# tlepoint/fhe.rs

Measured on NVIDIA H100. Metric: bfv_ct_mul_relin_per_sec_n32768_14x62bit, higher is better.
Workload: dtype u64

## Files before the change

### fhe_rs_b200/csrc/kernels.cu

```cuda
#include <algorithm>
#include <cstdint>
#include <cstdlib>
#include <cstring>

#include "engine.hpp"
#include "ntt_tma.cuh"

namespace fhe_b200 {

typedef unsigned __int128 u128;

namespace {

struct EwArgs {
  u64* a;
  const u64* b;
  size_t n_words;
  u32 logn, limbs_per_poly;
  const LimbDev* limbs;
  unsigned short ids[kMaxPos];
};

template <int OP>
__global__ void ew_kernel(EwArgs A) {
// ... 174 lines not shown
  size_t idx = (size_t)blockIdx.x * blockDim.x + threadIdx.x;
  size_t total = ((size_t)A.cts * nc * K) << A.logn;
  if (idx >= total) return;
  const u32 c = idx & (N - 1);
  size_t row = idx >> A.logn;
  const u32 pos = row % K;
  row /= K;
  const u32 k = row % nc, ct = (u32)(row / nc);
  const LimbDev& M = A.limbs[A.ids[pos]];
  const bool ext = pos >= A.L;
  const u32 rows = ext ? A.E : A.L, r = ext ? pos - A.L : pos;
  const u64* pa = (ext ? A.xa : A.a) + ((((size_t)ct * A.na) * rows + r) << A.logn) + c;
  const u64* pb = (ext ? A.xb : A.b) + ((((size_t)ct * A.nb) * rows + r) << A.logn) + c;
  const size_t ps = (size_t)rows << A.logn;
  Acc192 acc;
  acc.clear();
  const u32 lo = k + 1 > A.nb ? k + 1 - A.nb : 0, hi = k < A.na - 1 ? k : A.na - 1;
  for (u32 i = lo; i <= hi; i++) acc.mac(pa[i * ps], pb[(k - i) * ps]);
  A.out[idx] = acc.reduce(M);
}

struct ScaleArgs {
  ScalerDev S;
  const LimbDev* limbs;
  const u64* in;
  u64 *out0, *out1;
  u32 polys, out_rows_per_poly, start, n_out, split3, logn;
};

struct U256 {
  u64 w0, w1, w2, w3;
};
__device__ __forceinline__ U256 u256_from_acc(const u32 (&a)[7]) {
  U256 r;
  r.w0 = ((u64)a[1] << 32) | a[0];
  r.w1 = ((u64)a[3] << 32) | a[2];
  r.w2 = ((u64)a[5] << 32) | a[4];
  r.w3 = a[6];
  return r;
}
__device__ __forceinline__ U256 u256_add(U256 a, U256 b) {
  U256 r;
  asm("add.cc.u64 %0, %4, %8;\n\t"
      "addc.cc.u64 %1, %5, %9;\n\t"
      "addc.cc.u64 %2, %6, %10;\n\t"
      "addc.u64 %3, %7, %11;"
      : "=l"(r.w0), "=l"(r.w1), "=l"(r.w2), "=l"(r.w3)
      : "l"(a.w0), "l"(a.w1), "l"(a.w2), "l"(a.w3), "l"(b.w0), "l"(b.w1), "l"(b.w2), "l"(b.w3));
  return r;
}
__device__ __forceinline__ U256 u256_sub(U256 a, U256 b) {
  U256 r;
  asm("sub.cc.u64 %0, %4, %8;\n\t"
      "subc.cc.u64 %1, %5, %9;\n\t"
      "subc.cc.u64 %2, %6, %10;\n\t"
      "subc.u64 %3, %7, %11;"
      : "=l"(r.w0), "=l"(r.w1), "=l"(r.w2), "=l"(r.w3)
      : "l"(a.w0), "l"(a.w1), "l"(a.w2), "l"(a.w3), "l"(b.w0), "l"(b.w1), "l"(b.w2), "l"(b.w3));
  return r;
}
__device__ __forceinline__ U256 u256_mul_128(u128 v, u64 tlo, u64 thi) {
  u32 a[7] = {0, 0, 0, 0, 0, 0, 0}, b[7] = {0, 0, 0, 0, 0, 0, 0};
  mac_theta(a, (u64)v, tlo, thi);
  mac_theta(b, (u64)(v >> 64), tlo, thi);
  U256 lo = u256_from_acc(a), hi = u256_from_acc(b);
  U256 hs = {0, hi.w0, hi.w1, hi.w2};
  return u256_add(lo, hs);
}

constexpr int kScaleTC = 128;

__device__ __forceinline__ void stage_omega_split(u32* s_om, const ScalerDev& S, u32 start, u32 n_out, u32 n_out4) {
  const u32 nf = S.n_from;
  for (u32 idx = threadIdx.x; idx < nf * n_out4; idx += blockDim.x) {
    const u32 ii = idx / n_out4, jj = idx - ii * n_out4;
    const Split31 w = split31(jj < n_out ? S.omega[(size_t)(start + jj) * nf + ii] : 0);
    u32* row = s_om + (size_t)ii * 3 * n_out4 + jj;
    row[0] = w.lo;
    row[n_out4] = w.hi;
    row[2 * n_out4] = w.sum;
  }
}

template <int G, int UNR = 2>
__device__ __forceinline__ void scale_mac_group(AccKara (&acc)[4], const u64* r_col, const u32* om, u32 nf,
                                                u32 n_out4) {
#pragma unroll UNR
  for (u32 i = 0; i < nf; i++) {
    const Split31 r = split31(r_col[i * kScaleTC]);
    const u32* row = om + (size_t)i * 3 * n_out4;
    const uint4 w0 = *reinterpret_cast<const uint4*>(row);
    const uint4 w1 = *reinterpret_cast<const uint4*>(row + n_out4);
    const uint4 ws = *reinterpret_cast<const uint4*>(row + 2 * n_out4);
    acc[0].mac(r.lo, r.hi, r.sum, w0.x, w1.x, ws.x);
    if (G > 1) acc[1].mac(r.lo, r.hi, r.sum, w0.y, w1.y, ws.y);
    if (G > 2) acc[2].mac(r.lo, r.hi, r.sum, w0.z, w1.z, ws.z);
    if (G > 3) acc[3].mac(r.lo, r.hi, r.sum, w0.w, w1.w, ws.w);
  }
}

__global__ void __launch_bounds__(kScaleTC) scale_kernel(ScaleArgs A) {
  extern __shared__ __align__(16) u64 smem[];
  const ScalerDev& S = A.S;
  const u32 nf = S.n_from, n_out = A.n_out;
  const u32 n_out4 = (n_out + 3) & ~3u;
  constexpr u32 TC = kScaleTC;
  u64* s_r = smem;
  u32* s_omega = reinterpret_cast<u32*>(s_r + (size_t)nf * TC);
  u64* s_gamma = reinterpret_cast<u64*>(s_omega + (size_t)nf * 3 * n_out4);
  u64* s_tgl = s_gamma + n_out4;
  u64* s_tgh = s_tgl + nf;
  u64* s_tol = s_tgh + nf;
  u64* s_toh = s_tol + nf;
  u32* s_ord = reinterpret_cast<u32*>(s_toh + nf);

  const u32 N = 1u << A.logn;
  const u32 per_poly = N / TC;
  const u32 poly = blockIdx.x / per_poly;
  const u32 c0 = (blockIdx.x % per_poly) * TC;
  const u64* src = A.in + (((size_t)poly * nf) << A.logn) + c0;
  const u32 cc = threadIdx.x;

  {
    const u32 dst0 = (u32)__cvta_generic_to_shared(s_r + cc);
    for (u32 i = 0; i < nf; i++)
      asm volatile("cp.async.ca.shared.global [%0], [%1], 8;" ::"r"(dst0 + i * TC * 8u),
                   "l"(src + ((size_t)i << A.logn) + cc)
                   : "memory");
    asm volatile("cp.async.commit_group;" ::: "memory");
  }
  stage_omega_split(s_omega, S, A.start, n_out, n_out4);
  for (u32 i = cc; i < n_out4; i += TC) s_gamma[i] = i < n_out ? S.gamma[A.start + i] : 0;
  for (u32 i = cc; i < nf; i += TC) {
    s_tgl[i] = S.tgar_lo[i];
    s_tgh[i] = S.tgar_hi[i];
    s_tol[i] = S.to_lo[i];
    s_toh[i] = S.to_hi[i];
    s_ord[i] = i < S.n_terms ? S.to_order[i] : 0;
  }
  asm volatile("cp.async.wait_all;" ::: "memory");
  __syncthreads();

  u128 v;
  {
    AccTheta at;
    at.clear();
#pragma unroll 2
    for (u32 i = 0; i < nf; i++) at.mac(s_r[i * TC + cc], s_tgl[i], s_tgh[i]);
    u32 acc[7];
    at.words(acc);
    U256 sg = u256_from_acc(acc);
    const u32 bs = S.shift - 1 - 64;
    u64 lo = (sg.w1 >> bs) | (sg.w2 << (64 - bs));
    u64 hi = (sg.w2 >> bs) | (sg.w3 << (64 - bs));
    u128 x = ((u128)hi << 64) | lo;
    v = (x >> 1) + (x & 1);
  }
  bool w_sign = false;
  u128 w = 0;
  if (!S.is_one) {
    U256 s_pos = {0, 0, 0, 0}, s_neg = {0, 0, 0, 0};
#pragma unroll 1
    for (u32 sg = 0; sg < 2; sg++) {
      AccTheta at;
      at.clear();
      const u32 k0 = sg ? S.n_pos : 0, k1 = sg ? S.n_terms : S.n_pos;
#pragma unroll 2
      for (u32 k = k0; k < k1; k++) {
        const u32 i = s_ord[k];
        at.mac(s_r[i * TC + cc], s_tol[i], s_toh[i]);
      }
      u32 wds[7];
      at.words(wds);
      if (sg == 0) s_pos = u256_from_acc(wds);
      else s_neg = u256_from_acc(wds);
    }
    U256 so = u256_sub(s_pos, s_neg);
    U256 vt = u256_mul_128(v, S.tg_lo, S.tg_hi);
    so = S.tg_sign ? u256_add(so, vt) : u256_sub(so, vt);
    w_sign = (so.w3 != 0) || (so.w2 >> 63);
    if (w_sign) {
      u64 n1 = ~so.w1, n2 = ~so.w2, n3 = ~so.w3;
      u128 y = ((u128)((n2 >> 62) | (n3 << 2)) << 64) | ((n1 >> 62) | (n2 << 2));
      w = (y + 1) >> 1;
    } else {
      u128 y = ((u128)((so.w2 >> 62) | (so.w3 << 2)) << 64) | ((so.w1 >> 62) | (so.w2 << 2));
      w = (y >> 1) + (y & 1);
    }
  }

  for (u32 j0 = 0; j0 < n_out; j0 += 4) {
    AccKara acc[4];
#pragma unroll
    for (int k = 0; k < 4; k++) acc[k].clear();
    const u32* om = s_omega + j0;
    switch (min(4u, n_out - j0)) {
      case 4: scale_mac_group<4>(acc, s_r + cc, om, nf, n_out4); break;
      case 3: scale_mac_group<3>(acc, s_r + cc, om, nf, n_out4); break;
      case 2: scale_mac_group<2>(acc, s_r + cc, om, nf, n_out4); break;
      default: scale_mac_group<1>(acc, s_r + cc, om, nf, n_out4); break;
    }
#pragma unroll
    for (int k = 0; k < 4; k++) {
      const u32 jj = j0 + k;
      if (jj >= n_out) break;
      const LimbDev& M = A.limbs[S.to_ids[A.start + jj]];
      u64 vr = reduce94_limb((u64)v, (u64)(v >> 64), M);
      acc[k].mac(split31(vr ? M.p - vr : 0), split31(s_gamma[jj]));
      if (!S.is_one) {
        u64 wr = reduce94_limb((u64)w, (u64)(w >> 64), M);
        acc[k].add64(w_sign ? (wr ? M.p - wr : 0) : wr);
      }
      u64 y = acc[k].reduce(M);
      u64* dst;
      if (A.split3) {
        u32 ct = poly / 3, part = poly % 3;
        dst = part < 2 ? A.out0 + ((((size_t)ct * 2 + part) * n_out + jj) << A.logn)
                       : A.out1 + (((size_t)ct * n_out + jj) << A.logn);
      } else {
        dst = A.out0 + (((size_t)poly * A.out_rows_per_poly + jj) << A.logn);
      }
      dst[c0 + cc] = y;
    }
  }
}


struct ScaleTmaArgs {
  ScalerDev S;
  const LimbDev* limbs;
  u64 *out0, *out1;
  u32 polys, out_rows_per_poly, start, n_out, split3, logn;
  u32 tiles_total;
};

template <bool IS_ONE, int UNR>
__global__ void __launch_bounds__(kScaleTC) scale_tma_kernel(const __grid_constant__ CUtensorMap tm_in, const ScaleTmaArgs A) {
  using namespace tma;
  extern __shared__ __align__(128) u64 smem[];
  const ScalerDev& S = A.S;
  const u32 nf = S.n_from, n_out = A.n_out;
  const u32 n_out4 = (n_out + 3) & ~3u;
  constexpr u32 TC = kScaleTC;
  u64* s_r = smem;
  u32* s_omega = reinterpret_cast<u32*>(s_r + (size_t)nf * TC);
  u64* s_gamma = reinterpret_cast<u64*>(s_omega + (size_t)nf * 3 * n_out4);
  u64* s_p2 = s_gamma + n_out4;
  u64* s_c = s_p2 + n_out4;
  u64* s_tgl = s_c + n_out4;
  u64* s_tgh = s_tgl + nf;
  u64* s_tol = s_tgh + nf;
  u64* s_toh = s_tol + nf;
  u32* s_ord = reinterpret_cast<u32*>(s_toh + nf);
  u64* s_bar = reinterpret_cast<u64*>(s_ord + ((nf + 1) & ~1u));
  const u32 bar = smem_u32(s_bar);
  const u32 cc = threadIdx.x;

  stage_omega_split(s_omega, S, A.start, n_out, n_out4);
  for (u32 i = cc; i < n_out4; i += TC) {
    const bool live = i < n_out;
    const LimbDev& M = A.limbs[S.to_ids[A.start + (live ? i : 0)]];
    s_gamma[i] = live ? S.gamma[A.start + i] : 0;
    s_p2[i] = M.p2;
    s_c[i] = M.sol_c;
  }
  for (u32 i = cc; i < nf; i += TC) {
    s_tgl[i] = S.tgar_lo[i];
    s_tgh[i] = S.tgar_hi[i];
    const u32 src = (!IS_ONE && i < S.n_terms) ? S.to_order[i] : 0;
    s_tol[i] = IS_ONE ? 0 : S.to_lo[src];
    s_toh[i] = IS_ONE ? 0 : S.to_hi[src];
    s_ord[i] = src * TC * 8;
  }
  if (cc == 0) {
    mbar_init(bar, 1);
    asm volatile("fence.mbarrier_init.release.cluster;" ::: "memory");
  }
  __syncthreads();

  const u32 N = 1u << A.logn;
  const u32 per_poly = N / TC;
  const u32 dst_r = smem_u32(s_r);
  const u32 tile_bytes = nf * TC * 8;
  u32 tile = blockIdx.x;
  if (cc == 0 && tile < A.tiles_total) {
    mbar_expect_tx(bar, tile_bytes);
    load_2d(dst_r, &tm_in, (tile % per_poly) * TC, (tile / per_poly) * nf, bar);
  }
  const u32 my_r = dst_r + cc * 8;
  for (u32 it = 0; tile < A.tiles_total; tile += gridDim.x, it++) {
    const u32 poly = tile / per_poly;
    const u32 c0 = (tile - poly * per_poly) * TC;
    mbar_wait(bar, it & 1);

    u128 v;
    {
      AccTheta at;
      at.clear();
#pragma unroll 2
      for (u32 i = 0; i < nf; i++) at.mac(lds64(my_r + i * TC * 8), s_tgl[i], s_tgh[i]);
      u32 acc[7];
      at.words(acc);
      U256 sg = u256_from_acc(acc);
      const u32 bs = S.shift - 1 - 64;
      u64 lo = (sg.w1 >> bs) | (sg.w2 << (64 - bs));
      u64 hi = (sg.w2 >> bs) | (sg.w3 << (64 - bs));
      u128 x = ((u128)hi << 64) | lo;
      v = (x >> 1) + (x & 1);
    }
    bool w_sign = false;
    u128 w = 0;
    if (!IS_ONE) {
      U256 s_pos = {0, 0, 0, 0}, s_neg = {0, 0, 0, 0};
#pragma unroll 1
      for (u32 sg = 0; sg < 2; sg++) {
        AccTheta at;
        at.clear();
        const u32 k0 = sg ? S.n_pos : 0, k1 = sg ? S.n_terms : S.n_pos;
#pragma unroll 2
        for (u32 k = k0; k < k1; k++) at.mac(lds64(my_r + s_ord[k]), s_tol[k], s_toh[k]);
        u32 wds[7];
        at.words(wds);
        if (sg == 0) s_pos = u256_from_acc(wds);
        else s_neg = u256_from_acc(wds);
      }
      U256 so = u256_sub(s_pos, s_neg);
      U256 vt = u256_mul_128(v, S.tg_lo, S.tg_hi);
      so = S.tg_sign ? u256_add(so, vt) : u256_sub(so, vt);
      w_sign = (so.w3 != 0) || (so.w2 >> 63);
      if (w_sign) {
        u64 n1 = ~so.w1, n2 = ~so.w2, n3 = ~so.w3;
        u128 y = ((u128)((n2 >> 62) | (n3 << 2)) << 64) | ((n1 >> 62) | (n2 << 2));
        w = (y + 1) >> 1;
      } else {
        u128 y = ((u128)((so.w2 >> 62) | (so.w3 << 2)) << 64) | ((so.w1 >> 62) | (so.w2 << 2));
        w = (y >> 1) + (y & 1);
      }
    }
    const u64 mask62 = (1ull << 62) - 1;
    const u64 vl = (u64)v & mask62, wl = (u64)w & mask62;
    const u32 vh = (u32)(v >> 62), wh = (u32)(w >> 62);

    u64* dst;
    size_t dstride = (size_t)1 << A.logn;
    if (A.split3) {
      const u32 ct = poly / 3, part = poly - ct * 3;
      dst = part < 2 ? A.out0 + ((((size_t)ct * 2 + part) * n_out) << A.logn) : A.out1 + (((size_t)ct * n_out) << A.logn);
    } else {
      dst = A.out0 + (((size_t)poly * A.out_rows_per_poly) << A.logn);
    }
    dst += c0 + cc;

    for (u32 j0 = 0; j0 < n_out; j0 += 4) {
      AccKara acc[4];
#pragma unroll
      for (int k = 0; k < 4; k++) acc[k].clear();
      const u32* om = s_omega + j0;
      const u32 g = min(4u, n_out - j0);
      switch (g) {
        case 4: scale_mac_group<4, UNR>(acc, s_r + cc, om, nf, n_out4); break;
        case 3: scale_mac_group<3, UNR>(acc, s_r + cc, om, nf, n_out4); break;
        case 2: scale_mac_group<2, UNR>(acc, s_r + cc, om, nf, n_out4); break;
        default: scale_mac_group<1, UNR>(acc, s_r + cc, om, nf, n_out4); break;
      }
      if (j0 + 4 >= n_out) {
        __syncthreads();
        const u32 nxt = tile + gridDim.x;
        if (cc == 0 && nxt < A.tiles_total) {
          mbar_expect_tx(bar, tile_bytes);
          load_2d(dst_r, &tm_in, (nxt % per_poly) * TC, (nxt / per_poly) * nf, bar);
        }
      }
#pragma unroll
      for (int k = 0; k < 4; k++) {
        const u32 jj = j0 + k;
        if (jj >= n_out) break;
        const u64 p2 = s_p2[jj];
        const u32 c = (u32)s_c[jj];
        acc[k].mac(split31(csub(p2 - ((u64)vh * c + vl), p2 >> 1)), split31(s_gamma[jj]));
        if (!IS_ONE) {
          const u64 wr = (u64)wh * c + wl;
          acc[k].add64(w_sign ? p2 - wr : wr);
        }
        u64 lo, mid;
        u32 hi32;
        acc[k].merged(lo, mid, hi32);
        dst[(size_t)jj * dstride] = csub(fold192_solinas(lo, mid, hi32, c), p2 >> 1);
      }
    }
  }
}

__global__ void scale_small_kernel(ScaleArgs A) {
  const ScalerDev& S = A.S;
  const u32 nf = S.n_from, n_out = A.n_out;
  const u32 N = 1u << A.logn;
  const u32 idx = blockIdx.x * blockDim.x + threadIdx.x;
  if (idx >= A.polys * N) return;
  const u32 poly = idx >> A.logn, c = idx & (N - 1);
  const u64* src = A.in + (((size_t)poly * nf) << A.logn) + c;
  u32 av[7] = {0, 0, 0, 0, 0, 0, 0}, ap[7] = {0, 0, 0, 0, 0, 0, 0}, an[7] = {0, 0, 0, 0, 0, 0, 0};
  for (u32 i = 0; i < nf; i++) {
    const u64 r = src[(size_t)i << A.logn];
    mac_theta(av, r, S.tgar_lo[i], S.tgar_hi[i]);
    if (!S.is_one) {
      if (S.to_sign[i]) mac_theta(an, r, S.to_lo[i], S.to_hi[i]);
      else mac_theta(ap, r, S.to_lo[i], S.to_hi[i]);
    }
  }
  U256 sg = u256_from_acc(av);
  const u32 bs = S.shift - 1 - 64;
  u64 lo = (sg.w1 >> bs) | (sg.w2 << (64 - bs));
  u64 hi = (sg.w2 >> bs) | (sg.w3 << (64 - bs));
  u128 x = ((u128)hi << 64) | lo;
  u128 v = (x >> 1) + (x & 1);
  bool w_sign = false;
  u128 w = 0;
  if (!S.is_one) {
    U256 so = u256_sub(u256_from_acc(ap), u256_from_acc(an));
    U256 vt = u256_mul_128(v, S.tg_lo, S.tg_hi);
    so = S.tg_sign ? u256_add(so, vt) : u256_sub(so, vt);
    w_sign = (so.w3 != 0) || (so.w2 >> 63);
    if (w_sign) {
      u64 n1 = ~so.w1, n2 = ~so.w2, n3 = ~so.w3;
      u128 y = ((u128)((n2 >> 62) | (n3 << 2)) << 64) | ((n1 >> 62) | (n2 << 2));
      w = (y + 1) >> 1;
    } else {
      u128 y = ((u128)((so.w2 >> 62) | (so.w3 << 2)) << 64) | ((so.w1 >> 62) | (so.w2 << 2));
      w = (y >> 1) + (y & 1);
    }
  }
  for (u32 j = 0; j < n_out; j++) {
    const LimbDev& M = A.limbs[S.to_ids[A.start + j]];
    Acc192 acc;
    acc.clear();
    for (u32 i = 0; i < nf; i++) acc.mac(src[(size_t)i << A.logn], S.omega[(size_t)(A.start + j) * nf + i]);
    u64 vr = reduce128_limb((u64)v, (u64)(v >> 64), M);
    acc.mac(vr ? M.p - vr : 0, S.gamma[A.start + j]);
    if (!S.is_one) {
      u64 wr = reduce128_limb((u64)w, (u64)(w >> 64), M);
      acc.add64(w_sign ? (wr ? M.p - wr : 0) : wr);
    }
    u64 y = acc.reduce(M);
    u64* dst;
    if (A.split3) {
      u32 ct = poly / 3, part = poly % 3;
      dst = part < 2 ? A.out0 + ((((size_t)ct * 2 + part) * n_out + j) << A.logn)
                     : A.out1 + (((size_t)ct * n_out + j) << A.logn);
    } else {
      dst = A.out0 + (((size_t)poly * A.out_rows_per_poly + j) << A.logn);
    }
    dst[c] = y;
  }
}

struct KsMacArgs {
  const u64 *inter, *k0, *k1, *base0, *base1;
  u64 *out0, *out1;
  u32 cts, n_dig, Lk, out_ct_rows, logn;
  u32 adjacent;
  const LimbDev* limbs;
  unsigned short ids[kMaxPos];
};
__global__ void ksmac_kernel(KsMacArgs A) {
  const u32 N = 1u << A.logn;
  size_t idx = (size_t)blockIdx.x * blockDim.x + threadIdx.x;
  size_t total = ((size_t)A.cts * A.Lk) << A.logn;
  if (idx >= total) return;
  u32 c = idx & (N - 1);
  size_t row = idx >> A.logn;
// ... 710 lines not shown
  g_launches++;
}

void launch_mul_plain(u64* a, const u64* pt, u32 cts, u32 parts, u32 n_pt, const RowIds& ids, const LimbDev* limbs,
                      u32 logn, cudaStream_t st, u32 op) {
  MulPlainArgs A;
  A.a = a; A.pt = pt; A.cts = cts; A.parts = parts; A.n_pt = n_pt; A.logn = logn; A.op = op;
  A.limbs_per_poly = ids.limbs_per_poly; A.limbs = limbs;
  copy_ids(A.ids, ids);
  size_t total = ((size_t)cts * parts * ids.limbs_per_poly) << logn;
  if (!total) return;
  mul_plain_kernel<<<(unsigned)((total + 255) / 256), 256, 0, st>>>(A);
  g_launches++;
}

void launch_expand_butterfly(u64* lo, u64* hi, const u64* spill, u32 pairs, u32 n_hi, const ulonglong2* mono,
                             const RowIds& ids, const LimbDev* limbs, u32 logn, cudaStream_t st) {
  ExpandArgs A;
  const size_t ct_words = ((size_t)2 * ids.limbs_per_poly) << logn;
  A.lo = lo; A.hi = hi; A.spill = spill; A.mono = mono;
  A.n_words = pairs * ct_words;
  A.hi_words = n_hi * ct_words;
  A.logn = logn; A.limbs_per_poly = ids.limbs_per_poly; A.limbs = limbs;
  copy_ids(A.ids, ids);
  if (!A.n_words) return;
  const u32 threads = 256;
  expand_butterfly_kernel<<<(unsigned)((A.n_words / 2 + threads - 1) / threads), threads, 0, st>>>(A);
  g_launches++;
}

void launch_dot(const u64* ct, const u64* pt, u64* out, u32 groups, u32 n_terms, u32 parts, u32 ct_count,
                u32 pt_count, const RowIds& ids, const LimbDev* limbs, u32 logn, cudaStream_t st) {
  DotArgs A;
  A.ct = ct; A.pt = pt; A.out = out; A.groups = groups; A.n_terms = n_terms; A.parts = parts;
  A.ct_count = ct_count; A.pt_count = pt_count; A.logn = logn;
  A.limbs_per_poly = ids.limbs_per_poly; A.limbs = limbs;
  copy_ids(A.ids, ids);
  size_t total = ((size_t)groups * parts * ids.limbs_per_poly) << logn;
  if (!total) return;
  dot_kernel<<<(unsigned)((total + 255) / 256), 256, 0, st>>>(A);
  g_launches++;
}

void launch_tensor(const u64* a, const u64* b, const u64* xa, const u64* xb, u64* out, u32 cts, u32 L, u32 nca,
                   u32 ncb, u32 K, const RowIds& mul_ids, const LimbDev* limbs, u32 logn, cudaStream_t st) {
  TensorArgs A;
  A.a = a; A.b = b; A.xa = xa; A.xb = xb; A.out = out;
  A.cts = cts; A.L = L; A.nca = nca; A.ncb = ncb; A.K = K; A.logn = logn;
  A.limbs = limbs;
  copy_ids(A.ids, mul_ids);
  size_t total = ((size_t)cts * K) << logn;
  if (!total) return;
  tensor_kernel<<<(unsigned)((total + 255) / 256), 256, 0, st>>>(A);
  g_launches++;
}

void launch_tensor_nm(const u64* a, const u64* b, const u64* xa, const u64* xb, u64* out, u32 cts, u32 L, u32 E, u32 na,
                      u32 nb, const RowIds& mul_ids, const LimbDev* limbs, u32 logn, cudaStream_t st) {
  TensorNmArgs A;
  A.a = a; A.b = b; A.xa = xa; A.xb = xb; A.out = out;
  A.cts = cts; A.L = L; A.E = E; A.na = na; A.nb = nb; A.logn = logn;
  A.limbs = limbs;
  copy_ids(A.ids, mul_ids);
  size_t total = ((size_t)cts * (na + nb - 1) * (L + E)) << logn;
  if (!total) return;
  tensor_nm_kernel<<<(unsigned)((total + 255) / 256), 256, 0, st>>>(A);
  g_launches++;
}

static bool launch_scale_tma(const ScalerDev& S, const LimbDev* limbs, const u64* in, u64* out0, u64* out1, u32 polys,
                             u32 out_rows_per_poly, u32 start, u32 n_out, int split3, u32 logn, cudaStream_t st) {
  if (switches().classic_scaler || !tensor_map_encoder() || logn < 7 || (reinterpret_cast<uintptr_t>(in) & 127))
    return false;
  const u32 N = 1u << logn, nf = S.n_from;
  if (nf > 64 || (u64)polys * nf >= (1ull << 31)) return false;
  CUtensorMap tm;
  if (!box_map(&tm, in, (u64)polys * nf, logn, kScaleTC, nf)) return false;
  ScaleTmaArgs A;
  A.S = S; A.limbs = limbs; A.out0 = out0; A.out1 = out1;
  A.polys = polys; A.out_rows_per_poly = out_rows_per_poly; A.start = start; A.n_out = n_out;
  A.split3 = split3; A.logn = logn;
  A.tiles_total = polys * (N / kScaleTC);
  const size_t n_out4 = (n_out + 3) & ~(size_t)3;
  const size_t smem = (nf * kScaleTC + 3 * n_out4 + 4 * nf) * sizeof(u64) + nf * 3 * n_out4 * sizeof(u32) +
                      ((nf + 1) & ~(size_t)1) * 4 + 16;
  auto resident = [&](const void* k) {
    ensure_dynamic_smem(k, smem);
    int per_sm = 0;
    FHE_CUDA(cudaOccupancyMaxActiveBlocksPerMultiprocessor(&per_sm, k, kScaleTC, smem));
    return (u32)std::min<u64>(A.tiles_total, (u64)sm_count() * std::max(per_sm, 1));
  };
  if (switches().scale_unroll == 4) {
    if (S.is_one) scale_tma_kernel<true, 4><<<resident((const void*)scale_tma_kernel<true, 4>), kScaleTC, smem, st>>>(tm, A);
    else scale_tma_kernel<false, 4><<<resident((const void*)scale_tma_kernel<false, 4>), kScaleTC, smem, st>>>(tm, A);
  } else {
    if (S.is_one) scale_tma_kernel<true, 2><<<resident((const void*)scale_tma_kernel<true, 2>), kScaleTC, smem, st>>>(tm, A);
    else scale_tma_kernel<false, 2><<<resident((const void*)scale_tma_kernel<false, 2>), kScaleTC, smem, st>>>(tm, A);
  }
  g_launches++;
  return true;
}

void launch_scale(const ScalerDev& S, const LimbDev* limbs, const u64* in, u64* out0, u64* out1, u32 polys,
                  u32 out_rows_per_poly, u32 start, u32 n_out, int split3, u32 logn, cudaStream_t st) {
  if (!polys || !n_out) return;
  if (S.all_solinas &&
      launch_scale_tma(S, limbs, in, out0, out1, polys, out_rows_per_poly, start, n_out, split3, logn, st))
    return;
  ScaleArgs A;
  A.S = S; A.limbs = limbs; A.in = in; A.out0 = out0; A.out1 = out1;
  A.polys = polys; A.out_rows_per_poly = out_rows_per_poly; A.start = start; A.n_out = n_out;
  A.split3 = split3; A.logn = logn;
  const u32 N = 1u << logn;
  if (N < (u32)kScaleTC) {
    const u32 total = polys * N;
    scale_small_kernel<<<(total + 63) / 64, 64, 0, st>>>(A);
    g_launches++;
    return;
  }
  const size_t n_out4 = (n_out + 3) & ~(size_t)3, nf = S.n_from;
  const size_t smem = (nf * kScaleTC + n_out4 + 5 * nf) * sizeof(u64) + nf * 3 * n_out4 * sizeof(u32);
  ensure_dynamic_smem((const void*)scale_kernel, smem);
  scale_kernel<<<polys * (N / kScaleTC), kScaleTC, smem, st>>>(A);
  g_launches++;
}

void launch_ksmac(const u64* inter, const u64* k0, const u64* k1, const u64* base0, const u64* base1, u64* out0,
                  u64* out1, u32 cts, u32 n_dig, u32 Lk, u32 out_ct_rows, const RowIds& ids, const LimbDev* limbs,
                  u32 logn, cudaStream_t st, bool adjacent) {
  size_t total = ((size_t)cts * Lk) << logn;
  if (!total) return;
  const bool classic = switches().ksmac == Switches::KSMAC_CLASSIC;
  const int stages = (int)switches().ks_stages;
  const size_t smem_tma = ((size_t)(2 + stages) * n_dig * kKsTC + stages + 1) * sizeof(u64);
  if (adjacent && !classic && tensor_map_encoder() && logn >= 7 && n_dig <= 256 && smem_tma <= 200 * 1024 &&
      !((reinterpret_cast<uintptr_t>(inter) | reinterpret_cast<uintptr_t>(k0) | reinterpret_cast<uintptr_t>(k1)) & 127) &&
      (u64)cts * Lk * n_dig < (1ull << 31)) {
    CUtensorMap mt, m0, m1;
    if (box_map(&mt, inter, (u64)cts * Lk * n_dig, logn, kKsTC, n_dig) &&
        box_map(&m0, k0, (u64)Lk * n_dig, logn, kKsTC, n_dig) && box_map(&m1, k1, (u64)Lk * n_dig, logn, kKsTC, n_dig)) {
      KsTmaArgs T;
      T.base0 = base0; T.base1 = base1; T.out0 = out0; T.out1 = out1;
      T.cts = cts; T.n_dig = n_dig; T.Lk = Lk; T.out_ct_rows = out_ct_rows; T.logn = logn;
      T.items_total = Lk * ((1u << logn) / kKsTC) * cts;
      T.limbs = limbs;
      copy_ids(T.ids, ids);
      auto go = [&](auto kern) {
        ensure_dynamic_smem((const void*)kern, smem_tma);
        int per_sm = 0;
        FHE_CUDA(cudaOccupancyMaxActiveBlocksPerMultiprocessor(&per_sm, (const void*)kern, kKsTC, smem_tma));
        const u32 grid = (u32)std::min<u64>(T.items_total, (u64)sm_count() * std::max(per_sm, 1));
        kern<<<grid, kKsTC, smem_tma, st>>>(mt, m0, m1, T);
      };
      if (stages == 2) go(ksmac_tma_kernel<2>);
      else if (stages == 3) go(ksmac_tma_kernel<3>);
      else go(ksmac_tma_kernel<4>);
      g_launches++;
      return;
    }
  }
  KsMacArgs A;
  A.adjacent = adjacent ? 1 : 0;
  A.inter = inter; A.k0 = k0; A.k1 = k1; A.base0 = base0; A.base1 = base1; A.out0 = out0; A.out1 = out1;
  A.cts = cts; A.n_dig = n_dig; A.Lk = Lk; A.out_ct_rows = out_ct_rows; A.logn = logn;
  A.limbs = limbs;
  copy_ids(A.ids, ids);
  ksmac_kernel<<<(unsigned)((total + 255) / 256), 256, 0, st>>>(A);
// ... 54 lines not shown
```

### fhe_rs_b200/csrc/zq.cuh

```cuda
#pragma once
#include <cstdint>
#include <cuda_runtime.h>

namespace fhe_b200 {

typedef unsigned long long u64;
typedef unsigned int u32;

struct LimbDev {
  u64 p;
  u64 p2;
  u64 bhi;
  u64 blo;
  u64 ninv;
  u64 ninv_s;
  u64 zn;
  u64 zn_s;
  u64 c128;
  u64 sol_c;
  u64 sol_ntt;
  const ulonglong2* om;
  const ulonglong2* zi;
};

// ... 272 lines not shown
  __device__ __forceinline__ u64 reduce(const LimbDev& m) const {
    u64 lo, mid;
    u32 hi;
    merged(lo, mid, hi);
    return csub(reduce160_lazy(lo, mid, hi, m), m.p);
  }
};

struct Split31 {
  u32 lo, hi, sum;
};
__device__ __forceinline__ Split31 split31(u64 x) {
  const u32 lo = (u32)x & 0x7fffffffu, hi = (u32)(x >> 31);
  return {lo, hi, lo + hi};
}
struct AccKara {
  u64 l, m, h;
  u32 l2, m2, h2;
  __device__ __forceinline__ void clear() { l = m = h = 0; l2 = m2 = h2 = 0; }
  __device__ __forceinline__ void mac(u32 r0, u32 r1, u32 rs, u32 w0, u32 w1, u32 ws) {
    asm("{\n\t"
        ".reg .u32 x0, x1, y0, y1, z0, z1;\n\t"
        "mov.b64 {x0, x1}, %0;\n\t"
        "mov.b64 {y0, y1}, %1;\n\t"
        "mov.b64 {z0, z1}, %2;\n\t"
        "mad.lo.cc.u32 x0, %6, %9, x0;\n\t"
        "madc.hi.cc.u32 x1, %6, %9, x1;\n\t"
        "addc.u32 %3, %3, 0;\n\t"
        "mad.lo.cc.u32 y0, %8, %11, y0;\n\t"
        "madc.hi.cc.u32 y1, %8, %11, y1;\n\t"
        "addc.u32 %4, %4, 0;\n\t"
        "mad.lo.cc.u32 z0, %7, %10, z0;\n\t"
        "madc.hi.cc.u32 z1, %7, %10, z1;\n\t"
        "addc.u32 %5, %5, 0;\n\t"
        "mov.b64 %0, {x0, x1};\n\t"
        "mov.b64 %1, {y0, y1};\n\t"
        "mov.b64 %2, {z0, z1};\n\t"
        "}"
        : "+l"(l), "+l"(m), "+l"(h), "+r"(l2), "+r"(m2), "+r"(h2)
        : "r"(r0), "r"(r1), "r"(rs), "r"(w0), "r"(w1), "r"(ws));
  }
  __device__ __forceinline__ void mac(const Split31& r, const Split31& w) { mac(r.lo, r.hi, r.sum, w.lo, w.hi, w.sum); }
  __device__ __forceinline__ void add64(u64 v) {
    asm("add.cc.u64 %0, %0, %4;\n\t"
        "addc.u32 %1, %1, 0;\n\t"
        "add.cc.u64 %2, %2, %4;\n\t"
        "addc.u32 %3, %3, 0;"
        : "+l"(l), "+r"(l2), "+l"(m), "+r"(m2)
        : "l"(v));
  }
  __device__ __forceinline__ void merged(u64& lo, u64& mid, u32& hi) const {
    const u32 l0 = (u32)l, l1 = (u32)(l >> 32), h0 = (u32)h, h1 = (u32)(h >> 32);
    u32 d0, d1, d2;
    asm("sub.cc.u32 %0, %3, %6;\n\t"
        "subc.cc.u32 %1, %4, %7;\n\t"
        "subc.u32 %2, %5, %8;\n\t"
        "sub.cc.u32 %0, %0, %9;\n\t"
        "subc.cc.u32 %1, %1, %10;\n\t"
        "subc.u32 %2, %2, %11;"
        : "=r"(d0), "=r"(d1), "=r"(d2)
        : "r"((u32)m), "r"((u32)(m >> 32)), "r"(m2), "r"(l0), "r"(l1), "r"(l2), "r"(h0), "r"(h1), "r"(h2));
    const u32 a0 = d0 << 31, a1 = __funnelshift_l(d0, d1, 31), a2 = __funnelshift_l(d1, d2, 31), a3 = d2 >> 1;
    const u32 b1 = h0 << 30, b2 = __funnelshift_l(h0, h1, 30), b3 = __funnelshift_l(h1, h2, 30), b4 = h2 >> 2;
    u32 w0, w1, w2, w3;
    asm("add.cc.u32 %0, %5, %8;\n\t"
        "addc.cc.u32 %1, %6, %9;\n\t"
        "addc.cc.u32 %2, %7, %10;\n\t"
        "addc.cc.u32 %3, %11, 0;\n\t"
        "addc.u32 %4, %15, 0;\n\t"
        "add.cc.u32 %1, %1, %12;\n\t"
        "addc.cc.u32 %2, %2, %13;\n\t"
        "addc.cc.u32 %3, %3, %14;\n\t"
        "addc.u32 %4, %4, 0;"
        : "=r"(w0), "=r"(w1), "=r"(w2), "=r"(w3), "=r"(hi)
        : "r"(l0), "r"(l1), "r"(l2), "r"(a0), "r"(a1), "r"(a2), "r"(a3), "r"(b1), "r"(b2), "r"(b3), "r"(b4));
    lo = ((u64)w1 << 32) | w0;
    mid = ((u64)w3 << 32) | w2;
  }
  __device__ __forceinline__ u64 reduce(const LimbDev& m) const {
    u64 lo, mid;
    u32 hi;
    merged(lo, mid, hi);
    return csub(reduce160_lazy(lo, mid, hi, m), m.p);
  }
};

__device__ __forceinline__ u64 reduce128_limb(u64 lo, u64 hi, const LimbDev& m) {
  if (m.sol_c) return csub(fold192_solinas(lo, hi, 0, (u32)m.sol_c), m.p);
  return barrett128(lo, hi, m.p, m.bhi, m.blo);
}
__device__ __forceinline__ u64 reduce94_limb(u64 lo, u64 hi, const LimbDev& m) {
  if (m.sol_c) return csub(fold94_solinas(lo, hi, (u32)m.sol_c), m.p);
  return barrett128(lo, hi, m.p, m.bhi, m.blo);
}

__device__ __forceinline__ void mac_theta(u32 (&a)[7], u64 r, u64 tlo, u64 thi) {
  asm("{\n\t"
      ".reg .u32 r0, r1, t0, t1, t2, t3, u0, u1, u2, u3, u4, c;\n\t"
      ".reg .u64 P, C;\n\t"
      "mov.b64 {r0, r1}, %7;\n\t"
      "mov.b64 {t0, t1}, %8;\n\t"
      "mov.b64 {t2, t3}, %9;\n\t"
      "mul.wide.u32 P, r0, t0;\n\t"
      "mov.b64 {u0, c}, P;\n\t"
      "cvt.u64.u32 C, c;\n\t"
      "mad.wide.u32 P, r0, t1, C;\n\t"
      "mov.b64 {u1, c}, P;\n\t"
      "cvt.u64.u32 C, c;\n\t"
      "mad.wide.u32 P, r0, t2, C;\n\t"
      "mov.b64 {u2, c}, P;\n\t"
      "cvt.u64.u32 C, c;\n\t"
      "mad.wide.u32 P, r0, t3, C;\n\t"
      "mov.b64 {u3, u4}, P;\n\t"
      "add.cc.u32 %0, %0, u0;\n\t"
      "addc.cc.u32 %1, %1, u1;\n\t"
      "addc.cc.u32 %2, %2, u2;\n\t"
      "addc.cc.u32 %3, %3, u3;\n\t"
      "addc.cc.u32 %4, %4, u4;\n\t"
      "addc.cc.u32 %5, %5, 0;\n\t"
      "addc.u32 %6, %6, 0;\n\t"
      "mul.wide.u32 P, r1, t0;\n\t"
      "mov.b64 {u0, c}, P;\n\t"
      "cvt.u64.u32 C, c;\n\t"
      "mad.wide.u32 P, r1, t1, C;\n\t"
      "mov.b64 {u1, c}, P;\n\t"
      "cvt.u64.u32 C, c;\n\t"
      "mad.wide.u32 P, r1, t2, C;\n\t"
      "mov.b64 {u2, c}, P;\n\t"
      "cvt.u64.u32 C, c;\n\t"
      "mad.wide.u32 P, r1, t3, C;\n\t"
      "mov.b64 {u3, u4}, P;\n\t"
      "add.cc.u32 %1, %1, u0;\n\t"
      "addc.cc.u32 %2, %2, u1;\n\t"
      "addc.cc.u32 %3, %3, u2;\n\t"
      "addc.cc.u32 %4, %4, u3;\n\t"
      "addc.cc.u32 %5, %5, u4;\n\t"
      "addc.u32 %6, %6, 0;\n\t"
      "}"
      : "+r"(a[0]), "+r"(a[1]), "+r"(a[2]), "+r"(a[3]), "+r"(a[4]), "+r"(a[5]), "+r"(a[6])
      : "l"(r), "l"(tlo), "l"(thi));
}

struct AccTheta {
  u32 a[5], b[5], c[5], d[5];
  __device__ __forceinline__ void clear() {
#pragma unroll
    for (int i = 0; i < 5; i++) a[i] = b[i] = c[i] = d[i] = 0;
  }
  __device__ __forceinline__ void mac(u64 r, u64 tlo, u64 thi) {
    asm("{\n\t"
        ".reg .u32 r0, r1, t0, t1, t2, t3;\n\t"
        "mov.b64 {r0, r1}, %20;\n\t"
        "mov.b64 {t0, t1}, %21;\n\t"
        "mov.b64 {t2, t3}, %22;\n\t"
        "mad.lo.cc.u32 %0, r0, t0, %0;\n\t"
        "madc.hi.cc.u32 %1, r0, t0, %1;\n\t"
        "madc.lo.cc.u32 %2, r0, t2, %2;\n\t"
        "madc.hi.cc.u32 %3, r0, t2, %3;\n\t"
        "addc.u32 %4, %4, 0;\n\t"
        "mad.lo.cc.u32 %5, r0, t1, %5;\n\t"
        "madc.hi.cc.u32 %6, r0, t1, %6;\n\t"
        "madc.lo.cc.u32 %7, r0, t3, %7;\n\t"
        "madc.hi.cc.u32 %8, r0, t3, %8;\n\t"
        "addc.u32 %9, %9, 0;\n\t"
        "mad.lo.cc.u32 %10, r1, t0, %10;\n\t"
        "madc.hi.cc.u32 %11, r1, t0, %11;\n\t"
        "madc.lo.cc.u32 %12, r1, t2, %12;\n\t"
        "madc.hi.cc.u32 %13, r1, t2, %13;\n\t"
        "addc.u32 %14, %14, 0;\n\t"
        "mad.lo.cc.u32 %15, r1, t1, %15;\n\t"
        "madc.hi.cc.u32 %16, r1, t1, %16;\n\t"
        "madc.lo.cc.u32 %17, r1, t3, %17;\n\t"
        "madc.hi.cc.u32 %18, r1, t3, %18;\n\t"
        "addc.u32 %19, %19, 0;\n\t"
        "}"
        : "+r"(a[0]), "+r"(a[1]), "+r"(a[2]), "+r"(a[3]), "+r"(a[4]), "+r"(b[0]), "+r"(b[1]), "+r"(b[2]), "+r"(b[3]),
          "+r"(b[4]), "+r"(c[0]), "+r"(c[1]), "+r"(c[2]), "+r"(c[3]), "+r"(c[4]), "+r"(d[0]), "+r"(d[1]), "+r"(d[2]),
          "+r"(d[3]), "+r"(d[4])
        : "l"(r), "l"(tlo), "l"(thi));
  }
  __device__ __forceinline__ void words(u32 (&w)[7]) const {
    u64 t = (u64)a[1] + b[0] + c[0];
    w[0] = a[0];
    w[1] = (u32)t;
    t = (t >> 32) + a[2] + b[1] + c[1] + d[0];
    w[2] = (u32)t;
    t = (t >> 32) + a[3] + b[2] + c[2] + d[1];
    w[3] = (u32)t;
    t = (t >> 32) + a[4] + b[3] + c[3] + d[2];
    w[4] = (u32)t;
    t = (t >> 32) + b[4] + c[4] + d[3];
    w[5] = (u32)t;
    t = (t >> 32) + d[4];
    w[6] = (u32)t;
  }
};

__device__ __forceinline__ u64 mulmod_limb_lazy(u64 a, u64 b, const LimbDev& m) {
  if (m.sol_c) {
    u64 lo, hi;
    mul128_62(a, b, lo, hi);
    return fold192_solinas(lo, hi, 0, (u32)m.sol_c);
  }
  return barrett128_lazy(a * b, __umul64hi(a, b), m.p, m.bhi, m.blo);
}

__device__ __forceinline__ u64 mulmod_limb(u64 a, u64 b, const LimbDev& m) {
  if (m.sol_c) {
    u64 lo, hi;
    mul128_62(a, b, lo, hi);
    return csub(fold192_solinas(lo, hi, 0, (u32)m.sol_c), m.p);
  }
  return mulmod(a, b, m.p, m.bhi, m.blo);
}

}
```

Measured before the change: 3835.

## Fold the gamma correction into the scaler MAC loop and pack theta accumulators

For the IS_ONE scaler path, the per-output gamma correction term is folded into the MAC loop as an extra omega row holding -gamma mod p. A precomputed c*(-gamma) constant lets a new inline-asm Solinas reduction finish each output, replacing the separate gamma mac, merge and fold. It also adds minBlocks=6 launch bounds for UNR==2 and repacks the AccTheta accumulators into 64-bit pairs. This trades extra shared memory and register pressure for fewer per-output reduction instructions. A profiling script is added as well.

```diff
diff --git a/fhe_rs_b200/csrc/kernels.cu b/fhe_rs_b200/csrc/kernels.cu
--- a/fhe_rs_b200/csrc/kernels.cu
+++ b/fhe_rs_b200/csrc/kernels.cu
@@ -280,21 +280,27 @@
   }
 }
 
+template <int G>
+__device__ __forceinline__ void scale_mac_term(AccKara (&acc)[4], const Split31& r, const u32* row, u32 n_out4) {
+  const uint4 w0 = *reinterpret_cast<const uint4*>(row);
+  const uint4 w1 = *reinterpret_cast<const uint4*>(row + n_out4);
+  const uint4 ws = *reinterpret_cast<const uint4*>(row + 2 * n_out4);
+  acc[0].mac(r.lo, r.hi, r.sum, w0.x, w1.x, ws.x);
+  if (G > 1) acc[1].mac(r.lo, r.hi, r.sum, w0.y, w1.y, ws.y);
+  if (G > 2) acc[2].mac(r.lo, r.hi, r.sum, w0.z, w1.z, ws.z);
+  if (G > 3) acc[3].mac(r.lo, r.hi, r.sum, w0.w, w1.w, ws.w);
+}
 template <int G, int UNR = 2>
 __device__ __forceinline__ void scale_mac_group(AccKara (&acc)[4], const u64* r_col, const u32* om, u32 nf,
                                                 u32 n_out4) {
 #pragma unroll UNR
-  for (u32 i = 0; i < nf; i++) {
-    const Split31 r = split31(r_col[i * kScaleTC]);
-    const u32* row = om + (size_t)i * 3 * n_out4;
-    const uint4 w0 = *reinterpret_cast<const uint4*>(row);
-    const uint4 w1 = *reinterpret_cast<const uint4*>(row + n_out4);
-    const uint4 ws = *reinterpret_cast<const uint4*>(row + 2 * n_out4);
-    acc[0].mac(r.lo, r.hi, r.sum, w0.x, w1.x, ws.x);
-    if (G > 1) acc[1].mac(r.lo, r.hi, r.sum, w0.y, w1.y, ws.y);
-    if (G > 2) acc[2].mac(r.lo, r.hi, r.sum, w0.z, w1.z, ws.z);
-    if (G > 3) acc[3].mac(r.lo, r.hi, r.sum, w0.w, w1.w, ws.w);
-  }
+  for (u32 i = 0; i < nf; i++) scale_mac_term<G>(acc, split31(r_col[i * kScaleTC]), om + (size_t)i * 3 * n_out4, n_out4);
+}
+template <int G, int UNR>
+__device__ __forceinline__ void scale_mac_group_v(AccKara (&acc)[4], const u64* r_col, const u32* om, u32 nf,
+                                                  u32 n_out4, u64 vl) {
+  scale_mac_group<G, UNR>(acc, r_col, om, nf, n_out4);
+  scale_mac_term<G>(acc, split31(vl), om + (size_t)nf * 3 * n_out4, n_out4);
 }
 
 __global__ void __launch_bounds__(kScaleTC) scale_kernel(ScaleArgs A) {
@@ -433,7 +439,7 @@
 };
 
 template <bool IS_ONE, int UNR>
-__global__ void __launch_bounds__(kScaleTC) scale_tma_kernel(const __grid_constant__ CUtensorMap tm_in, const ScaleTmaArgs A) {
+__global__ void __launch_bounds__(kScaleTC, UNR == 2 ? 6 : 1) scale_tma_kernel(const __grid_constant__ CUtensorMap tm_in, const ScaleTmaArgs A) {
   using namespace tma;
   extern __shared__ __align__(128) u64 smem[];
   const ScalerDev& S = A.S;
@@ -442,10 +448,11 @@
   constexpr u32 TC = kScaleTC;
   u64* s_r = smem;
   u32* s_omega = reinterpret_cast<u32*>(s_r + (size_t)nf * TC);
-  u64* s_gamma = reinterpret_cast<u64*>(s_omega + (size_t)nf * 3 * n_out4);
-  u64* s_p2 = s_gamma + n_out4;
+  u64* s_p2 = reinterpret_cast<u64*>(s_omega + (size_t)(nf + 1) * 3 * n_out4);
   u64* s_c = s_p2 + n_out4;
-  u64* s_tgl = s_c + n_out4;
+  u64* s_ncg = s_c + n_out4;
+  u64* s_gamma = s_ncg + n_out4;
+  u64* s_tgl = s_gamma + n_out4;
   u64* s_tgh = s_tgl + nf;
   u64* s_tol = s_tgh + nf;
   u64* s_toh = s_tol + nf;
@@ -458,9 +465,18 @@
   for (u32 i = cc; i < n_out4; i += TC) {
     const bool live = i < n_out;
     const LimbDev& M = A.limbs[S.to_ids[A.start + (live ? i : 0)]];
-    s_gamma[i] = live ? S.gamma[A.start + i] : 0;
+    const u64 g = live ? S.gamma[A.start + i] % M.p : 0;
+    const u64 ng = g ? M.p - g : 0;
+    const u128 cng = (u128)M.sol_c * ng;
+    u32* row = s_omega + (size_t)nf * 3 * n_out4 + i;
+    const Split31 a = split31(ng);
+    row[0] = a.lo;
+    row[n_out4] = a.hi;
+    row[2 * n_out4] = a.sum;
     s_p2[i] = M.p2;
     s_c[i] = M.sol_c;
+    s_ncg[i] = reduce94_limb((u64)cng, (u64)(cng >> 64), M);
+    s_gamma[i] = live ? S.gamma[A.start + i] : 0;
   }
   for (u32 i = cc; i < nf; i += TC) {
     s_tgl[i] = S.tgar_lo[i];
@@ -555,11 +571,20 @@
       for (int k = 0; k < 4; k++) acc[k].clear();
       const u32* om = s_omega + j0;
       const u32 g = min(4u, n_out - j0);
-      switch (g) {
-        case 4: scale_mac_group<4, UNR>(acc, s_r + cc, om, nf, n_out4); break;
-        case 3: scale_mac_group<3, UNR>(acc, s_r + cc, om, nf, n_out4); break;
-        case 2: scale_mac_group<2, UNR>(acc, s_r + cc, om, nf, n_out4); break;
-        default: scale_mac_group<1, UNR>(acc, s_r + cc, om, nf, n_out4); break;
+      if (IS_ONE) {
+        switch (g) {
+          case 4: scale_mac_group_v<4, UNR>(acc, s_r + cc, om, nf, n_out4, vl); break;
+          case 3: scale_mac_group_v<3, UNR>(acc, s_r + cc, om, nf, n_out4, vl); break;
+          case 2: scale_mac_group_v<2, UNR>(acc, s_r + cc, om, nf, n_out4, vl); break;
+          default: scale_mac_group_v<1, UNR>(acc, s_r + cc, om, nf, n_out4, vl); break;
+        }
+      } else {
+        switch (g) {
+          case 4: scale_mac_group<4, UNR>(acc, s_r + cc, om, nf, n_out4); break;
+          case 3: scale_mac_group<3, UNR>(acc, s_r + cc, om, nf, n_out4); break;
+          case 2: scale_mac_group<2, UNR>(acc, s_r + cc, om, nf, n_out4); break;
+          default: scale_mac_group<1, UNR>(acc, s_r + cc, om, nf, n_out4); break;
+        }
       }
       if (j0 + 4 >= n_out) {
         __syncthreads();
@@ -575,15 +600,17 @@
         if (jj >= n_out) break;
         const u64 p2 = s_p2[jj];
         const u32 c = (u32)s_c[jj];
-        acc[k].mac(split31(csub(p2 - ((u64)vh * c + vl), p2 >> 1)), split31(s_gamma[jj]));
-        if (!IS_ONE) {
+        if (IS_ONE) {
+          dst[(size_t)jj * dstride] = acc[k].reduce_solinas(0, vh, s_ncg[jj], c, p2 >> 1);
+        } else {
+          acc[k].mac(split31(csub(p2 - ((u64)vh * c + vl), p2 >> 1)), split31(s_gamma[jj]));
           const u64 wr = (u64)wh * c + wl;
           acc[k].add64(w_sign ? p2 - wr : wr);
+          u64 lo, mid;
+          u32 hi32;
+          acc[k].merged(lo, mid, hi32);
+          dst[(size_t)jj * dstride] = csub(fold192_solinas(lo, mid, hi32, c), p2 >> 1);
         }
-        u64 lo, mid;
-        u32 hi32;
-        acc[k].merged(lo, mid, hi32);
-        dst[(size_t)jj * dstride] = csub(fold192_solinas(lo, mid, hi32, c), p2 >> 1);
       }
     }
   }
@@ -1460,7 +1487,7 @@
   A.split3 = split3; A.logn = logn;
   A.tiles_total = polys * (N / kScaleTC);
   const size_t n_out4 = (n_out + 3) & ~(size_t)3;
-  const size_t smem = (nf * kScaleTC + 3 * n_out4 + 4 * nf) * sizeof(u64) + nf * 3 * n_out4 * sizeof(u32) +
+  const size_t smem = (nf * kScaleTC + 4 * n_out4 + 4 * nf) * sizeof(u64) + (nf + 1) * 3 * n_out4 * sizeof(u32) +
                       ((nf + 1) & ~(size_t)1) * 4 + 16;
   auto resident = [&](const void* k) {
     ensure_dynamic_smem(k, smem);
diff --git a/fhe_rs_b200/csrc/zq.cuh b/fhe_rs_b200/csrc/zq.cuh
--- a/fhe_rs_b200/csrc/zq.cuh
+++ b/fhe_rs_b200/csrc/zq.cuh
@@ -378,6 +378,50 @@
     u32 hi;
     merged(lo, mid, hi);
     return csub(reduce160_lazy(lo, mid, hi, m), m.p);
+  }
+  __device__ __forceinline__ u64 reduce_solinas(u64 a, u32 b, u64 t, u32 c, u64 q) const {
+    u32 s0, s1, s2, s3;
+    asm("{\n\t"
+        ".reg .u32 d0, d1, d2, e0, e1, e2, e3;\n\t"
+        "sub.cc.u32 d0, %4, %7;\n\t"
+        "subc.cc.u32 d1, %5, %8;\n\t"
+        "subc.u32 d2, %6, %9;\n\t"
+        "sub.cc.u32 d0, d0, %10;\n\t"
+        "subc.cc.u32 d1, d1, %11;\n\t"
+        "subc.u32 d2, d2, %12;\n\t"
+        "shl.b32 e0, d0, 31;\n\t"
+        "shf.l.wrap.b32 e1, d0, d1, 31;\n\t"
+        "shf.l.wrap.b32 e2, d1, d2, 31;\n\t"
+        "shr.b32 e3, d2, 1;\n\t"
+        "add.cc.u32 %0, %7, %13;\n\t"
+        "addc.cc.u32 %1, %8, %14;\n\t"
+        "addc.u32 %2, %9, 0;\n\t"
+        "add.cc.u32 %0, %0, e0;\n\t"
+        "addc.cc.u32 %1, %1, e1;\n\t"
+        "addc.cc.u32 %2, %2, e2;\n\t"
+        "addc.u32 %3, e3, 0;\n\t"
+        "mad.lo.cc.u32 %0, %15, %10, %0;\n\t"
+        "madc.hi.cc.u32 %1, %15, %10, %1;\n\t"
+        "madc.lo.cc.u32 %2, %15, %12, %2;\n\t"
+        "madc.hi.u32 %3, %15, %12, %3;\n\t"
+        "mad.lo.cc.u32 %1, %15, %11, %1;\n\t"
+        "madc.hi.cc.u32 %2, %15, %11, %2;\n\t"
+        "addc.u32 %3, %3, 0;\n\t"
+        "mad.lo.cc.u32 %0, %16, %17, %0;\n\t"
+        "madc.hi.cc.u32 %1, %16, %17, %1;\n\t"
+        "addc.cc.u32 %2, %2, 0;\n\t"
+        "addc.u32 %3, %3, 0;\n\t"
+        "mad.lo.cc.u32 %1, %16, %18, %1;\n\t"
+        "madc.hi.cc.u32 %2, %16, %18, %2;\n\t"
+        "addc.u32 %3, %3, 0;\n\t"
+        "}"
+        : "=&r"(s0), "=&r"(s1), "=&r"(s2), "=&r"(s3)
+        : "r"((u32)m), "r"((u32)(m >> 32)), "r"(m2), "r"((u32)l), "r"((u32)(l >> 32)), "r"(l2), "r"((u32)h),
+          "r"((u32)(h >> 32)), "r"(h2), "r"((u32)a), "r"((u32)(a >> 32)), "r"(c), "r"(b), "r"((u32)t),
+          "r"((u32)(t >> 32)));
+    u64 lo = ((u64)s1 << 32) | s0, hi = ((u64)s3 << 32) | s2;
+    fold_step_solinas(lo, hi, 0, c);
+    return csub(fold94_solinas(lo, hi, c), q);
   }
 };
 
@@ -437,45 +481,43 @@
       : "l"(r), "l"(tlo), "l"(thi));
 }
 
+#define FHE_THETA_CHAIN(LO, HI, TOP, RW, TA, TB)                                        \
+"mov.b64 {x0, x1}, " LO ";\n\t"                                                 \
+"mov.b64 {x2, x3}, " HI ";\n\t"                                                 \
+"mad.lo.cc.u32 x0, " RW ", " TA ", x0;\n\t"                                      \
+"madc.hi.cc.u32 x1, " RW ", " TA ", x1;\n\t"                                     \
+"madc.lo.cc.u32 x2, " RW ", " TB ", x2;\n\t"                                     \
+"madc.hi.cc.u32 x3, " RW ", " TB ", x3;\n\t"                                     \
+"addc.u32 " TOP ", " TOP ", 0;\n\t"                                             \
+"mov.b64 " LO ", {x0, x1};\n\t"                                                 \
+"mov.b64 " HI ", {x2, x3};\n\t"
 struct AccTheta {
-  u32 a[5], b[5], c[5], d[5];
+  u64 a01, a23, b01, b23, c01, c23, d01, d23;
+  u32 a4, b4, c4, d4;
   __device__ __forceinline__ void clear() {
-#pragma unroll
-    for (int i = 0; i < 5; i++) a[i] = b[i] = c[i] = d[i] = 0;
+    a01 = a23 = b01 = b23 = c01 = c23 = d01 = d23 = 0;
+    a4 = b4 = c4 = d4 = 0;
   }
   __device__ __forceinline__ void mac(u64 r, u64 tlo, u64 thi) {
     asm("{\n\t"
-        ".reg .u32 r0, r1, t0, t1, t2, t3;\n\t"
-        "mov.b64 {r0, r1}, %20;\n\t"
-        "mov.b64 {t0, t1}, %21;\n\t"
-        "mov.b64 {t2, t3}, %22;\n\t"
-        "mad.lo.cc.u32 %0, r0, t0, %0;\n\t"
-        "madc.hi.cc.u32 %1, r0, t0, %1;\n\t"
-        "madc.lo.cc.u32 %2, r0, t2, %2;\n\t"
-        "madc.hi.cc.u32 %3, r0, t2, %3;\n\t"
-        "addc.u32 %4, %4, 0;\n\t"
-        "mad.lo.cc.u32 %5, r0, t1, %5;\n\t"
-        "madc.hi.cc.u32 %6, r0, t1, %6;\n\t"
-        "madc.lo.cc.u32 %7, r0, t3, %7;\n\t"
-        "madc.hi.cc.u32 %8, r0, t3, %8;\n\t"
-        "addc.u32 %9, %9, 0;\n\t"
-        "mad.lo.cc.u32 %10, r1, t0, %10;\n\t"
-        "madc.hi.cc.u32 %11, r1, t0, %11;\n\t"
-        "madc.lo.cc.u32 %12, r1, t2, %12;\n\t"
-        "madc.hi.cc.u32 %13, r1, t2, %13;\n\t"
-        "addc.u32 %14, %14, 0;\n\t"
-        "mad.lo.cc.u32 %15, r1, t1, %15;\n\t"
-        "madc.hi.cc.u32 %16, r1, t1, %16;\n\t"
-        "madc.lo.cc.u32 %17, r1, t3, %17;\n\t"
-        "madc.hi.cc.u32 %18, r1, t3, %18;\n\t"
-        "addc.u32 %19, %19, 0;\n\t"
+        ".reg .u32 r0, r1, t0, t1, t2, t3, x0, x1, x2, x3;\n\t"
+        "mov.b64 {r0, r1}, %12;\n\t"
+        "mov.b64 {t0, t1}, %13;\n\t"
+        "mov.b64 {t2, t3}, %14;\n\t"
+        FHE_THETA_CHAIN("%0", "%1", "%8", "r0", "t0", "t2")
+        FHE_THETA_CHAIN("%2", "%3", "%9", "r0", "t1", "t3")
+        FHE_THETA_CHAIN("%4", "%5", "%10", "r1", "t0", "t2")
+        FHE_THETA_CHAIN("%6", "%7", "%11", "r1", "t1", "t3")
         "}"
-        : "+r"(a[0]), "+r"(a[1]), "+r"(a[2]), "+r"(a[3]), "+r"(a[4]), "+r"(b[0]), "+r"(b[1]), "+r"(b[2]), "+r"(b[3]),
-          "+r"(b[4]), "+r"(c[0]), "+r"(c[1]), "+r"(c[2]), "+r"(c[3]), "+r"(c[4]), "+r"(d[0]), "+r"(d[1]), "+r"(d[2]),
-          "+r"(d[3]), "+r"(d[4])
+        : "+l"(a01), "+l"(a23), "+l"(b01), "+l"(b23), "+l"(c01), "+l"(c23), "+l"(d01), "+l"(d23), "+r"(a4), "+r"(b4),
+          "+r"(c4), "+r"(d4)
         : "l"(r), "l"(tlo), "l"(thi));
   }
   __device__ __forceinline__ void words(u32 (&w)[7]) const {
+    const u32 a[5] = {(u32)a01, (u32)(a01 >> 32), (u32)a23, (u32)(a23 >> 32), a4};
+    const u32 b[5] = {(u32)b01, (u32)(b01 >> 32), (u32)b23, (u32)(b23 >> 32), b4};
+    const u32 c[5] = {(u32)c01, (u32)(c01 >> 32), (u32)c23, (u32)(c23 >> 32), c4};
+    const u32 d[5] = {(u32)d01, (u32)(d01 >> 32), (u32)d23, (u32)(d23 >> 32), d4};
     u64 t = (u64)a[1] + b[0] + c[0];
     w[0] = a[0];
     w[1] = (u32)t;
diff --git a/profiles/scaler_bench.py b/profiles/scaler_bench.py
--- /dev/null
+++ b/profiles/scaler_bench.py
@@ -0,0 +1,173 @@
+import argparse
+import json
+import os
+import re
+import shutil
+import subprocess
+import sys
+import tempfile
+import threading
+
+os.environ.setdefault("FHE_B200_STREAMS", "1")
+ROOT = os.path.dirname(os.path.dirname(os.path.abspath(__file__)))
+sys.path.insert(0, ROOT)
+import numpy as np
+import torch
+from torch.profiler import ProfilerActivity, profile
+
+import fhe_rs_b200 as F
+from bench import DEGREE, N_MODULI, PLAINTEXT, fill_uniform
+
+RECORDED_MAC_RATE = 25.0
+
+
+def scaler_imad_wide(n_from, n_out, n_w):
+    return 3 * n_from * n_out + 8 * (n_from + n_w)
+
+
+SHAPES = {"scale_tma_kernel<true, 2>": (14, 15, 0), "scale_tma_kernel<false, 2>": (29, 14, 14)}
+
+
+def smi(fields):
+    q = subprocess.run(["nvidia-smi", "--query-gpu=" + fields, "--format=csv,noheader,nounits", "-i", "0"],
+                       capture_output=True, text=True, timeout=30, check=True)
+    return [x.strip() for x in q.stdout.strip().split(",")]
+
+
+class ClockSampler:
+
+    def __init__(self):
+        self.samples, self._stop = [], threading.Event()
+        self._t = threading.Thread(target=self._run, daemon=True)
+
+    def _run(self):
+        p = subprocess.Popen(["nvidia-smi", "--query-gpu=clocks.sm", "--format=csv,noheader,nounits", "-i", "0",
+                              "-lms", "100"], stdout=subprocess.PIPE, text=True)
+        try:
+            for line in p.stdout:
+                if line.strip().isdigit():
+                    self.samples.append(int(line))
+                if self._stop.is_set():
+                    break
+        finally:
+            p.terminate()
+            p.wait()
+
+    def __enter__(self):
+        self._t.start()
+        return self
+
+    def __exit__(self, *a):
+        self._stop.set()
+        self._t.join(timeout=10)
+
+    def mhz(self):
+        s = sorted(self.samples)
+        return s[len(s) // 2] if s else None
+
+
+def mac_bench_rate():
+    nvcc = shutil.which("nvcc") or "/usr/local/cuda/bin/nvcc"
+    if not os.path.exists(nvcc):
+        return None, None
+    with tempfile.TemporaryDirectory() as d:
+        exe = os.path.join(d, "mac_bench")
+        r = subprocess.run([nvcc, "-gencode", "arch=compute_90a,code=sm_90a", "-O3", "-std=c++17", "-o", exe,
+                            os.path.join(ROOT, "bench_micro", "mac_bench.cu")], capture_output=True, text=True)
+        if r.returncode != 0:
+            return None, None
+        with ClockSampler() as cs:
+            out = subprocess.run([exe], capture_output=True, text=True, check=True).stdout
+    nominal = int(smi("clocks.max.sm")[0])
+    for line in out.splitlines():
+        m = re.match(r"V3 NACC=4 warps/SMSP= 6 : +([\d.]+) ms -> +([\d.]+) clk", line)
+        if m:
+            clk = float(m.group(2)) * (cs.mhz() or nominal) / nominal
+            return 3 * 32 * 4 / clk, out
+    return None, out
+
+
+def profiled(op, steps):
+    op()
+    torch.cuda.synchronize()
+    with profile(activities=[ProfilerActivity.CUDA]) as prof:
+        for _ in range(steps):
+            op()
+        torch.cuda.synchronize()
+    per = {}
+    for ev in prof.events():
+        if ev.device_type != torch.autograd.DeviceType.CUDA or "scale_tma_kernel" not in ev.name:
+            continue
+        k = "scale_tma_kernel<true, 2>" if "<true" in ev.name else "scale_tma_kernel<false, 2>"
+        per[k] = per.get(k, 0.0) + ev.time_range.elapsed_us() / 1e3 / steps
+    return per
+
+
+def main():
+    ap = argparse.ArgumentParser()
+    ap.add_argument("batch", nargs="?", type=int, default=256)
+    ap.add_argument("--steps", type=int, default=3)
+    ap.add_argument("--mac-rate", type=float, help="loop rate to compare against when mac_bench cannot be built")
+    ap.add_argument("--json", help="also write the results as JSON")
+    a = ap.parse_args()
+    assert torch.cuda.is_available(), "scaler_bench.py needs a CUDA device"
+
+    name, plim, maxclk = smi("name,power.limit,clocks.max.sm")
+    sms = torch.cuda.get_device_properties(0).multi_processor_count
+    rate, src = mac_bench_rate()
+    if rate is None:
+        rate = a.mac_rate or RECORDED_MAC_RATE
+        src = "mac_bench could not be built here: loop rate %.1f taken from %s" % (
+            rate, "--mac-rate" if a.mac_rate else "DESIGN section 3.3")
+    else:
+        src = "loop rate measured now with bench_micro/mac_bench.cu (V3, NACC=4, 6 warps/SMSP)"
+
+    par = F.BfvParameters(DEGREE, PLAINTEXT, moduli_sizes=[62] * N_MODULI, device=0)
+    moduli = par.moduli()
+    A, B = F.Ciphertext(par, a.batch, 2), F.Ciphertext(par, a.batch, 2)
+    fill_uniform(torch, A, moduli, 1)
+    fill_uniform(torch, B, moduli, 2)
+    rng = np.random.default_rng(7)
+    kc = np.zeros((2, N_MODULI, N_MODULI, DEGREE), np.uint64)
+    for i, q in enumerate(moduli):
+        kc[:, :, i, :] = rng.integers(0, q, size=(2, N_MODULI, DEGREE), dtype=np.uint64)
+    m = F.Multiplicator.default(F.RelinearizationKey.from_arrays(par, kc[0], kc[1]))
+    X = F.Ciphertext(par, a.batch, 2, mul_basis=True)
+    fill_uniform(torch, X, par.mul_basis(0), 3)
+
+    def mul():
+        m.multiply(A, B).sync()
+
+    with ClockSampler() as cs:
+        in_product = profiled(mul, a.steps)
+        direct = profiled(lambda: (A.scale(0), X.scale(1)), a.steps)
+    mhz = cs.mhz() or int(maxclk)
+    coeffs = a.batch * DEGREE
+    polys = {"scale_tma_kernel<true, 2>": (4, 2), "scale_tma_kernel<false, 2>": (3, 2)}
+    print("%s, power limit %s W, SM clock %d MHz (median of %d samples, max %s); %d SMs; batch %d, %d steps, "
+          "FHE_B200_STREAMS=%s" % (name, plim, mhz, len(cs.samples), maxclk, sms, a.batch, a.steps,
+                                   os.environ["FHE_B200_STREAMS"]))
+    print("%s: %.1f lane-IMAD.WIDE per SM per clock" % (src, rate))
+    print("%-28s %-11s %9s %11s %14s %9s" % ("kernel", "route", "ms/step", "IMAD.W/coef", "IMAD.W/SM/clk",
+                                            "of loop"))
+    rows = []
+    for k, (nf, no, nw) in SHAPES.items():
+        per_coef = scaler_imad_wide(nf, no, nw)
+        for route, table, np_ in (("product", in_product, polys[k][0]), ("scale()", direct, polys[k][1])):
+            ms = table.get(k)
+            if ms is None:
+                continue
+            achieved = per_coef * coeffs * np_ / (ms * 1e-3 * sms * mhz * 1e6)
+            rows.append({"kernel": k, "route": route, "ms_per_step": ms, "imad_wide_per_coef": per_coef,
+                         "polys_per_step": np_ * a.batch, "imad_wide_per_sm_clk": achieved,
+                         "fraction_of_loop": achieved / rate})
+            print("%-28s %-11s %9.3f %11d %14.2f %8.1f%%" % (k, route, ms, per_coef, achieved, 100 * achieved / rate))
+    if a.json:
+        with open(a.json, "w") as f:
+            json.dump({"gpu": name, "power_limit_w": float(plim), "sm_clock_mhz": mhz, "sms": sms,
+                       "batch": a.batch, "steps": a.steps, "loop_rate": rate, "loop_rate_source": src,
+                       "kernels": rows}, f, indent=1)
+
+
+if __name__ == "__main__":
+    main()
```

After: 3887 (median of 6 runs). +1.3%, better.
